# HipGraph/Force2Vec

Hardware: AMD Instinct MI355X
Metric: embedding edges/sec at D=128, option 5 (higher is better)
Workload: dtype f32; 1 GPU; RMAT scale-20 edge-factor 16 (n=1048576, nnz=31404412 directed CSR nonzeros), option 5, D=128, ns=5, lr=0.02, batch=65536; step = 1 epoch; batch=65536, hub_chunk=128, parallelism=1 GPU, recoveries=0, merge_finalize=1

## Files before the change

### force2vec_amd/_lib.py

```python
import ctypes as C
import os

HERE = os.path.dirname(os.path.abspath(__file__))
LIB_PATH = os.path.join(HERE, "libf2v.so")
SELFTEST_LIB_PATH = os.path.join(HERE, "libf2v_selftest.so")

F2V_OK, F2V_EINVAL, F2V_ENODEV, F2V_ENOMEM, F2V_EIO, F2V_ESTATE = 0, -1, -2, -3, -4, -5
INIT_SYMMETRIC, INIT_UNIT = 0, 1
SIM_DOT, SIM_L2, SIM_COSINE = 0, 1, 2
NEAREST_MAX_K = 128
NEAREST_EXCLUDE_SELF, NEAREST_EXCLUDE_NEIGHBOURS = 1, 2
NEAREST_PAD_ID = 0xFFFFFFFF
KMEANS_MAX_K, KMEANS_PIECE = 1024, 64

u32p = C.POINTER(C.c_uint32)
f32p = C.POINTER(C.c_float)


class Stats(C.Structure):
    _fields_ = [("step_launches", C.c_uint64), ("rows", C.c_uint64), ("nnz", C.c_uint64),
                ("algorithmic_bytes", C.c_uint64), ("device_seconds", C.c_double),
                ("hub_rows", C.c_uint64), ("hub_chunks", C.c_uint64), ("compulsory_bytes", C.c_uint64),
                ("snapshot_seconds", C.c_double), ("recoveries", C.c_uint64), ("recovered", C.c_uint32), ("merge_finalize", C.c_uint32)]

# ... 55 lines not shown
    "f2v_push_masks": (C.c_int, [u32p, u32p, C.c_uint32, C.c_uint32, C.c_uint32, u32p, C.c_uint64, u32p]),
    "f2v_push_stats": (C.c_int, [C.c_void_p, C.POINTER(C.c_uint64), C.POINTER(C.c_uint64)]),
    "f2v_read_mtx": (C.c_int, [C.c_char_p, u32p, C.POINTER(C.c_uint64), C.POINTER(u32p), C.POINTER(u32p)]),
    "f2v_free": (None, [C.c_void_p]),
    "f2v_write_embd": (C.c_int, [C.c_char_p, f32p, C.c_uint32, C.c_uint32]),
    "f2v_write_csr_bin": (C.c_int, [C.c_char_p, u32p, u32p, C.c_uint32, C.c_uint64]),
    "f2v_read_csr_bin": (C.c_int, [C.c_char_p, u32p, C.POINTER(C.c_uint64), C.POINTER(u32p), C.POINTER(u32p)]),
    "f2v_write_embd_bin": (C.c_int, [C.c_char_p, f32p, C.c_uint32, C.c_uint32]),
    "f2v_read_embd": (C.c_int, [C.c_char_p, u32p, u32p, C.POINTER(f32p)]),
    "f2v_read_embd_bin": (C.c_int, [C.c_char_p, C.c_uint32, C.c_uint32, f32p]),
    "f2v_output_name": (C.c_int, [C.c_char_p, C.c_char_p, C.c_int, C.c_int, C.c_uint32, C.c_uint32, C.c_uint32, C.c_uint32, C.c_char_p, C.c_size_t]),
    "f2v_rng_create": (C.c_void_p, [C.c_uint32]),
    "f2v_rng_destroy": (None, [C.c_void_p]),
    "f2v_rng_next": (C.c_int, [C.c_void_p]),
    "f2v_rng_jump": (None, [C.c_void_p, C.c_uint64]),
    "f2v_rng_fill": (C.c_int, [C.c_void_p, f32p, C.c_uint64, C.c_int]),
    "f2v_rng_walks": (C.c_int, [C.c_void_p, u32p, u32p, C.c_uint32, C.c_uint64, u32p]),
    "f2v_sm_table": (C.c_int, [f32p]),
    "f2v_diag_ipc_preflight": (C.c_int, [C.c_int, C.c_uint32, C.c_uint32, C.c_char_p, C.c_uint64, C.c_double]),
    "f2v_diag_stream_copy": (C.c_int, [C.c_int, C.c_uint64, C.c_uint32, C.POINTER(C.c_double)]),
    "f2v_diag_gather_rate": (C.c_int, [C.c_int, C.c_uint64, C.c_uint32, C.POINTER(C.c_double)]),
}

TEST_SIGNATURES = {
    "f2v_test_push_attach_local": (C.c_int, [C.c_void_p, C.c_uint32, C.c_uint32, C.POINTER(C.c_void_p)]),
    "f2v_test_gather_calibration": (C.c_int, [C.c_int, C.c_uint32, C.c_uint32]),
    "f2v_test_wave_reduce": (C.c_int, [C.c_int, f32p, C.c_uint32, C.c_uint32, f32p]),
    "f2v_test_withhold_flag": (C.c_int, [C.c_void_p, C.c_uint32]),
    "f2v_test_chain_nowait": (C.c_int, [C.c_void_p, C.c_int]),
    "f2v_test_withhold_row": (C.c_int, [C.c_void_p, C.c_uint32]),
    "f2v_test_stamps": (C.c_int, [C.c_void_p, C.c_int, C.POINTER(C.c_uint64)]),
    "f2v_test_xcd_times": (C.c_int, [C.c_void_p, C.c_int, C.POINTER(C.c_uint64)]),
    "f2v_test_plan_gather": (C.c_int, [C.c_void_p, C.c_uint32, C.c_uint32, C.c_uint32, C.c_uint32, C.POINTER(C.c_double)]),
    "f2v_test_wide_plan_check": (C.c_int, [u32p, u32p, C.c_uint32, C.c_uint64, C.c_uint32, C.c_uint32, C.c_int, C.POINTER(C.c_char_p), C.POINTER(C.c_int64), C.c_uint32, C.POINTER(C.c_uint64)]),
}

PUSH_EXPORT_BYTES = 256
PUSH_MAX_RANKS = 8

_lib = None
_selftest = None


class F2VError(RuntimeError):
    def __init__(self, code, msg):
        super().__init__("libf2v error %d: %s" % (code, msg))
        self.code = code


def lib():
    global _lib
    if _lib is None:
        path = os.environ.get("F2V_LIBRARY", LIB_PATH)
        if not os.path.exists(path):
            raise ImportError("%s is missing: build it with `make` (hipcc --offload-arch=gfx950); "
                              "force2vec_amd has no fallback implementation" % path)
        L = C.CDLL(path)
        for name, (res, args) in SIGNATURES.items():
            if path != LIB_PATH and not hasattr(L, name):
                continue
            fn = getattr(L, name)
            fn.restype = res
            fn.argtypes = args
        _lib = L
    return _lib

# ... 21 lines not shown
```

### force2vec_amd/csrc/f2v_engine.hip

```cpp
#include <hip/hip_runtime.h>

#include <algorithm>
#include <chrono>
#include <cstdio>
#include <cstdlib>
#include <cstring>
#include <functional>
#include <condition_variable>
#include <map>
#include <mutex>
#include <memory>
#include <string>
#include <atomic>
#include <thread>
#include <tuple>
#include <type_traits>
#include <vector>

#include "f2v.h"
#ifdef F2V_TEST_HOOKS
#include "f2v_test.h"
#endif
#include "f2v_internal.h"
#include "f2v_kernels.hip.h"
// ... 107 lines not shown
    std::vector<double> loss_values;
    struct Nearest {
        float *d_Q = nullptr, *d_rq = nullptr, *d_rc = nullptr, *d_scores = nullptr;
        uint32_t *d_qids = nullptr, *d_ids = nullptr;
        unsigned long long *d_ws = nullptr, *d_counts = nullptr;
        size_t q_cap = 0, ws_cap = 0, out_cap = 0;
        hipEvent_t ev[2] = {nullptr, nullptr};
        uint32_t splits = 0, block = 0, chunk = 8192;
        uint32_t lds_allowed = 0;
    } nn;
    int rows_sorted = -1;
    struct Kmeans {
        float *d_C = nullptr, *d_bestC = nullptr, *d_dist = nullptr;
        uint32_t *d_labels = nullptr, *d_bestL = nullptr, *d_order = nullptr, *d_hist = nullptr, *d_counts = nullptr, *d_start = nullptr,
                 *d_pstart = nullptr, *d_changed = nullptr, *d_seed = nullptr, *d_mlabels = nullptr;
        double *d_psum = nullptr, *d_ipart = nullptr, *d_inertia = nullptr;
        unsigned long long *d_tallies = nullptr;
        uint32_t cap_k = 0, cap_nc = 0;
        hipEvent_t ev[2] = {nullptr, nullptr};
        uint32_t block = 0;
        uint32_t lds_allowed = 0;
    } km;
    uint32_t last_wide_width = 0;
    bool last_wide_early = false;
    int last_train_form = 0;
    bool plan_overflow = false;
    uint32_t *h_kerr = nullptr;
#ifdef F2V_TEST_HOOKS
    uint32_t test_withhold_slot = kNoSlot, test_withhold_row = kNoSlot;
    uint32_t test_chain_mode = 0;
    bool test_chain_nowait = false;
    unsigned long long *d_xcd = nullptr;
    unsigned long long *d_stamps = nullptr;
#endif
    bool merge_fin = true, capturing = false;
    int cur = 0;
    bool have_x = false, have_walks = false;
    bool x_invalid = false;
    Rand rng;
    uint32_t chunk = 64, fanin = 32;
    bool chunk_auto = true;
    bool use_quarter = true;
    std::map<std::tuple<uint32_t, uint32_t, int>, Plan> plans;
    std::map<std::tuple<uint32_t, uint32_t, uint32_t, int>, ChainPlan> chains;
    std::vector<WgDesc> h_wg;
    WgDesc *d_wg = nullptr;
    size_t d_wg_cap = 0, d_wg_valid = 0;
    std::map<std::tuple<uint32_t, uint32_t, uint32_t, int>, WidePlan> wides;
    PlanVec<WideDesc> h_wide;
    PlanVec<WJob> h_jobs;
    WideDesc *d_wide = nullptr;
    WJob *d_jobs = nullptr;
    size_t d_wide_cap = 0, d_wide_valid = 0, d_jobs_cap = 0, d_jobs_valid = 0;
    bool wide = true;
    uint32_t wide_max_batch = 2048;
    uint32_t wide_rows = 262144;
    uint32_t wide_order = 0;
    uint32_t wide_phases = 1;
    uint32_t wide_min_width = 0;
    uint32_t wide_epochs = 0, last_wide_epochs = 1;
    float *d_ring = nullptr, *d_ring_partials = nullptr;
    uint32_t *d_ring_flags = nullptr, *d_ring_ready = nullptr;
    uint32_t ring_epochs = 0;
    bool ring_refused = false;
    size_t ring_slots = 0;
    bool wide_single = false;
// ... 1172 lines not shown
    c->stats.compulsory_bytes += plan.compulsory * epochs;
}

void scale_stats(f2v_stats &s, uint64_t epochs, uint64_t per) {
    for (uint64_t *v : {&s.step_launches, &s.rows, &s.nnz, &s.algorithmic_bytes, &s.hub_rows, &s.hub_chunks, &s.compulsory_bytes}) *v = *v / per * epochs;
}

FinalizeArgs finalize_args(const f2v_ctx *c, const StepArgs &a, const FinItem *items, uint32_t n) {
    FinalizeArgs f{};
    f.X = a.X;
    f.partials = c->d_partials;
    f.Xn = a.Xn;
    f.items = items;
    f.n_items = n;
    f.D = c->D;
    f.push = a.push;
    return f;
}

int launch_step(f2v_ctx *c, int math, uint32_t batch_lo, uint32_t batch_hi, uint32_t row_lo, uint32_t row_hi,
                const uint32_t *d_ids, uint32_t ns, float lr, int bs_mode, bool push = false, const uint32_t *push_masks = nullptr) {
    int rc;
    if ((rc = flush_unless_continued(c, batch_lo)) != F2V_OK) return rc;
    const Plan plan = plan_for(c, row_lo, row_hi, math == 7);
    if ((rc = upload_plans(c)) != F2V_OK) return rc;
    StepArgs a{};
    fill_step_args(c, a, math, plan.item_off, c->upd_lo, ns, lr, bs_mode);
    a.sample_ids = d_ids;
    a.batch_lo = batch_lo;
    a.n_items = plan.n_items;
    a.upd_rows = c->upd_hi - c->upd_lo;
#ifdef F2V_TEST_HOOKS
    a.xcd_times = c->d_xcd;
#endif
    push = push && c->push.attached && c->push.world > 1;
    if (push) fill_targets(c, a.push, c->cur ^ 1, batch_lo, push_masks);

    const uint32_t wpb = (uint32_t)c->waves_per_block;
    const uint32_t width = subwave_width(c);
    const bool quarter = width != 0;
    const uint32_t per_wave = items_per_wave(width);
    const uint32_t waves = (plan.n_items + per_wave - 1) / per_wave;
    uint32_t blocks = (waves + wpb - 1) / wpb;
    a.step_blocks = blocks;
    uint32_t tree_nodes = 0;
    for (int lev = 0; lev < plan.n_levels; lev++) tree_nodes += plan.fin_cnt[lev];
    const bool fused_tree = quarter && c->merge_fin && !c->capturing && plan.n_levels >= 1 && blocks > 0;
    if (fused_tree) {
        a.fin_items = c->d_hubs + plan.fin_off[0];
        a.fin_n = tree_nodes;
        arm_waits(c, a, false);
        blocks += (a.fin_n + wpb - 1) / wpb;
    }
    if (blocks == 0) {
    } else if (quarter) {
        rc = dispatch_subwave<16, true>(c, math, width, [&](auto O, auto L, auto N, auto U, auto FL) {
            constexpr int OPT = decltype(O)::value, LPI = decltype(L)::value, NB = decltype(N)::value, UR = decltype(U)::value;
            constexpr bool FULL = decltype(FL)::value;
            if (push) hipLaunchKernelGGL((qstep_kernel<OPT, LPI, NB, UR, true, FULL>), dim3(blocks), dim3(64 * wpb), 0, c->stream, a);
            else hipLaunchKernelGGL((qstep_kernel<OPT, LPI, NB, UR, false, FULL>), dim3(blocks), dim3(64 * wpb), 0, c->stream, a);
        });
        if (rc != F2V_OK) return rc;
    } else {
        rc = dispatch_math_layout(c, math, [&](auto O, auto V, auto E) {
            hipLaunchKernelGGL((step_kernel<decltype(O)::value, decltype(V)::value, decltype(E)::value>), dim3(blocks), dim3(64 * wpb), 0, c->stream, a);
        });
// ... 1969 lines not shown
        }
        hipError_t he = hipIpcOpenMemHandle((void **)&c->push.peer_flags[r], e.flags, hipIpcMemLazyEnablePeerAccess);
        if (he != hipSuccess) {
            c->push.peer_flags[r] = nullptr;
            (void)push_detach(c);
            return fail(F2V_ENODEV, "f2v_push_attach: cannot map the flags of rank %u: %s", r, hipGetErrorString(he));
        }
    }
    c->push.mask_batch = 0;
    c->push.exported = false;
    return F2V_OK;
}

#ifdef F2V_TEST_HOOKS
int f2v_test_withhold_flag(f2v_handle c, uint32_t slot) {
    if (!c) return fail(F2V_EINVAL, "null handle");
    c->test_withhold_slot = slot;
    return F2V_OK;
}

int f2v_test_withhold_row(f2v_handle c, uint32_t row) {
    if (!c) return fail(F2V_EINVAL, "null handle");
    c->test_withhold_row = row;
    return F2V_OK;
}

int f2v_test_chain_nowait(f2v_handle c, int on) {
    if (!c) return fail(F2V_EINVAL, "null handle");
    c->test_chain_nowait = (on & 1) != 0;
    c->test_chain_mode = (uint32_t)on;
    return F2V_OK;
}

int f2v_test_wide_plan_check(const uint32_t *rowptr, const uint32_t *colids, uint32_t n, uint64_t nnz, uint32_t dim, uint32_t batch, int walk,
                             const char *const *names, const int64_t *values, uint32_t n_params, uint64_t *stats_out) {
    if (!rowptr || (!colids && nnz) || n < 2 || dim == 0 || batch == 0) return fail(F2V_EINVAL, "f2v_test_wide_plan_check: bad argument");
    f2v_ctx ctx;
    f2v_ctx *c = &ctx;
    unsigned plan_threads = 0;
    c->n = n; c->nnz = nnz; c->D = dim;
    c->rowptr.assign(rowptr, rowptr + n + 1);
    c->colids.assign(colids, colids + nnz);
    c->chunk = auto_chunk(c, batch);
    static const char *const planner_reads[] = {"hub_chunk", "hub_fanin", "class_cut", "wide_phases", "wide_rounds", "wide_span", "wide_finish", "wide_order", "wide_rows", "wide_min_width"};
    for (uint32_t k = 0; k < n_params; k++) {
        const char *nm = names[k];
        if (!strcmp(nm, "plan_threads")) plan_threads = (unsigned)values[k];
        else if (std::any_of(std::begin(planner_reads), std::end(planner_reads), [&](const char *r) { return !strcmp(r, nm); })) find_param(nm)->put(c, values[k]);
        else return fail(F2V_EINVAL, "f2v_test_wide_plan_check: unknown parameter '%s'", nm);
    }
    if (!wide_usable(c) || subwave_width(c) == 0) return fail(F2V_EINVAL, "f2v_test_wide_plan_check: the wide form does not run this shape");
    const uint32_t nb = (uint32_t)(((uint64_t)n + batch - 1) / batch), K = chain_len(c, batch, true);
    const uint32_t width = wide_width(c, batch), ipb = wide_items_per_block(width), pslots = std::max<uint32_t>(ipb, 32u), F = c->fanin;
    std::vector<uint32_t> finished(n, 0), covered(nnz, 0);
    uint64_t st[7] = {};
    if (plan_threads) wide_plans_for_epoch(c, nb, K, batch, walk != 0, plan_threads);
#define F2V_PLAN_FAIL(...) return fail(F2V_ESTATE, "f2v_test_wide_plan_check: " __VA_ARGS__)
    for (uint32_t b0 = 0; b0 < nb; b0 += K) {
        const WidePlan p = wide_plan_for(c, b0, std::min(K, nb - b0), batch, walk != 0);
        if (c->plan_overflow) F2V_PLAN_FAIL("slot overflow");
        st[0] += p.n_wgs; st[1] += p.n_helpers; st[2] += p.n_finishers; st[3] += p.n_packed; st[4] += p.n_node_wgs; st[5] = std::max<uint64_t>(st[5], p.n_slots);
        std::vector<int64_t> producer(p.n_slots + 1, -1);
        uint32_t last_lo = 0;
        for (uint32_t wgi = 0; wgi < p.n_wgs; wgi++) {
            const WideDesc &d = c->h_wide[p.wg_off + wgi];
            if (d.kind == 0) {
// ... 469 lines not shown
```

### force2vec_amd/csrc/f2v_kernels.hip.h

```cpp
#ifndef F2V_KERNELS_HIP_H_
#define F2V_KERNELS_HIP_H_

#include <hip/hip_runtime.h>
#include <stdint.h>

namespace f2v {
#ifdef F2V_TEST_HOOKS
inline namespace selftest {
#endif

struct Item {
    uint32_t row;
    uint32_t nb;
    uint32_t cnt;
    uint32_t flags;
};
constexpr uint32_t kItemPartial = 1u << 31;
constexpr uint32_t kItemFirst = 1u << 30;
constexpr uint32_t kItemLast = 1u << 29;
constexpr uint32_t kItemSlotMask = (1u << 28) - 1;

struct FinItem {
    uint32_t in_slot, n;
    uint32_t out;
// ... 13 lines not shown
struct StepArgs {
    const float *X;
    float *Xn;
    const uint32_t *rowptr;
    const uint32_t *nbr_ids;
    float *partials;
    const uint32_t *sample_ids;
    const Item *items;
    const float *sm_table;
    uint32_t D;
    uint32_t batch_lo;
    uint32_t n_items;
    uint32_t upd_lo, upd_rows;
    uint32_t ns;
    uint32_t bs_mode;
    uint32_t unit_degi;
    float lr;
    PushTargets push;
    const FinItem *fin_items;
    uint32_t fin_n;
    uint32_t step_blocks;
    uint32_t seq;
    uint32_t *ready;
    uint32_t *err;
    unsigned long long timeout_ticks;
    uint32_t *rowflag;
    uint32_t chain_lo, chain_rows;
#ifdef F2V_TEST_HOOKS
    uint32_t test_withhold_slot;
    unsigned long long *stamps;
    uint32_t test_withhold_row;
    uint32_t test_nowait;
    unsigned long long *xcd_times;
#endif
};
constexpr uint32_t kNoSlot = 0xFFFFFFFFu;

struct FinalizeArgs {
    const float *X;
    float *partials;
    float *Xn;
    const FinItem *items;
    uint32_t n_items;
    uint32_t D;
    PushTargets push;
};

template <int CTRL>
__device__ __forceinline__ float dpp_mov(float v) {
    return __builtin_bit_cast(float, __builtin_amdgcn_update_dpp(0, __builtin_bit_cast(int, v), CTRL, 0xF, 0xF, true));
}

__device__ __forceinline__ float wave_allreduce_tree(float v) {
    v = v + dpp_mov<0xB1>(v);
    v = v + dpp_mov<0x4E>(v);
    v = v + dpp_mov<0x141>(v);
    v = v + dpp_mov<0x140>(v);
    v = v + __builtin_bit_cast(float, __builtin_amdgcn_ds_swizzle(__builtin_bit_cast(int, v), 0x401F));
    const float lo = __builtin_bit_cast(float, __builtin_amdgcn_readlane(__builtin_bit_cast(int, v), 0));
    const float hi = __builtin_bit_cast(float, __builtin_amdgcn_readlane(__builtin_bit_cast(int, v), 32));
    return lo + hi;
}

template <int VEC>
__device__ __forceinline__ float inlane_tree(float (&t)[VEC]) {
#pragma unroll
// ... 489 lines not shown

template <int OPT, int LPI, int NB, bool NEG>
__device__ __forceinline__ void pair_apply_q(const float (&xi)[NB][4], const float4 (&xj4)[NB], float (&Y)[NB][4], float lr,
                                             typename PairCoef<OPT, NEG>::type coef) {
    float xj[NB][4];
#pragma unroll
    for (int b = 0; b < NB; ++b) {
        xj[b][0] = xj4[b].x; xj[b][1] = xj4[b].y; xj[b][2] = xj4[b].z; xj[b][3] = xj4[b].w;
    }
#pragma unroll
    for (int b = 0; b < NB; ++b) {
#pragma unroll
        for (int v = 0; v < 4; ++v) {
            if constexpr (OPT == 5) {
                const float f = clamp_ref((xi[b][v] - xj[b][v]) * coef);
                const float s = lr * f;
                Y[b][v] = Y[b][v] + s;
            } else if constexpr (!NEG) {
                Y[b][v] = (float)((double)xj[b][v] * coef + (double)Y[b][v]);
            } else {
                const float p = coef * xj[b][v];
                Y[b][v] = Y[b][v] - p;
            }
        }
    }
}

template <int OPT, int LPI, int NB, bool NEG>
__device__ __forceinline__ void pair_update_q(const float (&xi)[NB][4], const float4 (&xj4)[NB], float (&Y)[NB][4],
                                              float lr, double c0, const float *table) {
    pair_apply_q<OPT, LPI, NB, NEG>(xi, xj4, Y, lr, pair_coef_q<OPT, LPI, NB, NEG>(xi, xj4, lr, c0, table));
}

__device__ __forceinline__ bool wait_row_slow(const StepArgs &a, const uint32_t *flags, uint32_t j) {
    const uint32_t *f = flags + j;
    const unsigned long long t0 = wall_clock64();
    for (uint32_t spins = 1;; ++spins) {
        __builtin_amdgcn_s_sleep(1);
        if (__hip_atomic_load(f, __ATOMIC_RELAXED, __HIP_MEMORY_SCOPE_AGENT) == a.seq) {
#ifdef F2V_TEST_HOOKS
            if (a.stamps) atomicMax(a.stamps + 4 * (size_t)j + 3, ~wall_clock64());
#endif
            return false;
        }
        if ((spins & 15u) != 0u) continue;
        if (__hip_atomic_load(a.err, __ATOMIC_RELAXED, __HIP_MEMORY_SCOPE_AGENT) != 0u) return true;
        if (wall_clock64() - t0 > a.timeout_ticks) {
            if (__hip_atomic_fetch_add(a.err + 1, 1u, __ATOMIC_RELAXED, __HIP_MEMORY_SCOPE_AGENT) == 0u) {
                a.err[2] = blockIdx.x; a.err[3] = j; a.err[4] = *f; a.err[5] = a.seq; a.err[6] = gridDim.x; a.err[7] = a.batch_lo;
            }
            __hip_atomic_store(a.err, 3u, __ATOMIC_RELAXED, __HIP_MEMORY_SCOPE_AGENT);
            return true;
        }
    }
}

__device__ __forceinline__ bool wait_row_at(const StepArgs &a, const uint32_t *flags, uint32_t j) {
    bool bad = false;
    if (__hip_atomic_load(flags + j, __ATOMIC_RELAXED, __HIP_MEMORY_SCOPE_AGENT) != a.seq) bad = wait_row_slow(a, flags, j);
    asm volatile("" ::: "memory");
    return bad;
}
__device__ __forceinline__ bool wait_row(const StepArgs &a, uint32_t j) { return wait_row_at(a, a.rowflag, j); }

__device__ __forceinline__ const float *row_src(const StepArgs &a, uint32_t j, uint32_t D) {
    return ((j - a.upd_lo) < a.upd_rows ? a.Xn : a.X) + (size_t)j * D;
}

typedef __amdgpu_buffer_rsrc_t rsrc_t;
__device__ __forceinline__ rsrc_t hand_rsrc(const float *base) {
    return __builtin_amdgcn_make_buffer_rsrc(const_cast<float *>(base), 0, -1, 0x00020000);
}
__device__ __forceinline__ float4 load16_agent(rsrc_t r, uint32_t byte_off) {
    const f32x4_t v = __builtin_bit_cast(f32x4_t, __builtin_amdgcn_raw_buffer_load_b128(r, (int)byte_off, 0,  16));
    return make_float4(v.x, v.y, v.z, v.w);
}
struct HandSrc {
    rsrc_t r;
    uint32_t xn_off, x_off, row_bytes;
    __device__ __forceinline__ uint32_t at(uint32_t j, bool second) const { return j * row_bytes + (second ? xn_off : x_off); }
};
__device__ __forceinline__ HandSrc hand_src_window(const StepArgs &a, uint32_t D) {
    HandSrc h;
    h.r = hand_rsrc(a.Xn + (size_t)a.chain_lo * D);
    h.row_bytes = D * 4u;
    h.xn_off = 0u - a.chain_lo * h.row_bytes;
    h.x_off = 0u;
    return h;
}

template <int OPT, int LPI, int NB, bool NEG, int U, bool FULL, bool CHAIN>
__device__ __forceinline__ void qprocess(const StepArgs &a, const HandSrc &hs, const uint32_t *ids, const uint32_t *idle, uint32_t cnt, uint32_t maxcnt,
                                         uint32_t t, uint32_t D, const float (&xi)[NB][4], float (&Y)[NB][4], double c0, const float *table, bool &bad) {
    constexpr bool kAllInFlight = !CHAIN && !(OPT != 5 && !FULL && U == 4);
    if constexpr (kAllInFlight) {
        const uint32_t last = cnt != 0u ? cnt - 1u : 0u;
        const uint32_t *list = cnt != 0u ? ids : idle;
        uint32_t j[U];
#pragma unroll
        for (int u = 0; u < U; ++u) j[u] = list[(uint32_t)u < last ? (uint32_t)u : last];
        for (uint32_t g = 0; g < maxcnt; g += U) {
            float4 xj[U][NB];
#pragma unroll
            for (int u = 0; u < U; ++u) {
                const float *src = row_src(a, j[u], D);
#pragma unroll
                for (int b = 0; b < NB; ++b) {
                    if constexpr (FULL) {
                        xj[u][b] = *reinterpret_cast<const float4 *>(src + t * 4 + 4 * LPI * b);
                    } else {
                        const bool live = 4u * LPI * b + 4u * t < D;
                        const float4 v = *reinterpret_cast<const float4 *>(src + (live ? t * 4 + 4 * LPI * b : 0u));
                        xj[u][b] = live ? v : make_float4(0.f, 0.f, 0.f, 0.f);
                    }
                }
            }
#pragma unroll
            for (int u = 0; u < U; ++u) {
                const uint32_t k = g + U + u;
                j[u] = list[k < last ? k : last];
            }
            asm volatile("" ::: "memory");
#pragma unroll
            for (int u = 0; u < U; ++u) {
                if (g + u < cnt) pair_update_q<OPT, LPI, NB, NEG>(xi, xj[u], Y, a.lr, c0, table);
            }
        }
        return;
    }
    uint32_t j[U];
#pragma unroll
    for (int u = 0; u < U; ++u) j[u] = ((uint32_t)u < cnt) ? ids[u] : 0u;
    for (uint32_t g = 0; g < maxcnt; g += U) {
        float4 xj[U][NB];
#pragma unroll
        for (int u = 0; u < U; ++u) {
            if (g + u < cnt) {
                bool handed = false;
                if constexpr (CHAIN) {
                    handed = (j[u] - a.chain_lo) < a.chain_rows;
                    if (handed) bad = wait_row(a, j[u]) || bad;
                }
                const float *src = row_src(a, j[u], D) + t * 4;
#pragma unroll
                for (int b = 0; b < NB; ++b) {
                    if (!(FULL || 4u * LPI * b + 4u * t < D)) xj[u][b] = make_float4(0.f, 0.f, 0.f, 0.f);
                    else if (CHAIN && handed) xj[u][b] = load16_agent(hs.r, hs.at(j[u], true) + 16u * t + 16u * LPI * b);
                    else xj[u][b] = *reinterpret_cast<const float4 *>(src + 4 * LPI * b);
                }
            }
        }
#pragma unroll
        for (int u = 0; u < U; ++u) j[u] = (g + U + u < cnt) ? ids[g + U + u] : 0u;
#pragma unroll
        for (int u = 0; u < U; ++u) {
            if (g + u < cnt) pair_update_q<OPT, LPI, NB, NEG>(xi, xj[u], Y, a.lr, c0, table);
        }
    }
// ... 185 lines not shown
    if (active) it = a.items[idx];
    else { it.row = 0; it.nb = 0; it.cnt = 0; it.flags = 0; }
    const uint32_t row = it.row;
    const bool partial = (it.flags & kItemPartial) != 0;
    const bool first_chunk = (it.flags & kItemFirst) != 0;
    const bool last_chunk = (it.flags & kItemLast) != 0;

    float xi[NB][4], Y[NB][4];
    {
        const float *src = a.X + (size_t)row * D + t * 4;
#pragma unroll
        for (int b = 0; b < NB; ++b) {
            const float4 v = (FULL || 4u * LPI * b + 4u * t < D) ? *reinterpret_cast<const float4 *>(src + 4 * LPI * b) : make_float4(0.f, 0.f, 0.f, 0.f);
            xi[b][0] = v.x; xi[b][1] = v.y; xi[b][2] = v.z; xi[b][3] = v.w;
        }
    }
    double c0 = 0.0;
    if constexpr (OPT == 5) {
#pragma unroll
        for (int b = 0; b < NB; ++b)
#pragma unroll
            for (int v = 0; v < 4; ++v) Y[b][v] = 0.0f;
    } else {
#pragma unroll
        for (int b = 0; b < NB; ++b)
#pragma unroll
            for (int v = 0; v < 4; ++v) Y[b][v] = first_chunk ? xi[b][v] : 0.0f;
        const uint32_t gdeg = a.rowptr[row + 1] - a.rowptr[row];
        const float degi = a.unit_degi ? 1.0f : (float)(1.0 / (double)(gdeg + 1u));
        c0 = (double)(a.lr * degi);
    }

    bool bad = false;
    const uint32_t *idle = &a.items[active ? idx : IPW * w].row;
    qprocess<OPT, LPI, NB, false, U, FULL, CHAIN>(a, hs, a.nbr_ids + it.nb, idle, it.cnt, wave_max_of_items<LPI>(it.cnt), t, D, xi, Y, c0, table, bad);
    if (lds_samples) {
        if (active && last_chunk) {
            for (uint32_t sidx = 0; sidx < a.ns; ++sidx) {
                float4 xs[NB];
#pragma unroll
                for (int b = 0; b < NB; ++b) xs[b] = smp[sidx][LPI * b + t];
                pair_update_q<OPT, LPI, NB, true>(xi, xs, Y, a.lr, c0, table);
            }
        }
    } else {
        const uint32_t scnt = (active && last_chunk) ? a.ns : 0u;
        const uint32_t sbase = a.bs_mode ? (row - a.batch_lo) : 0u;
        qprocess<OPT, LPI, NB, true, U, FULL, CHAIN>(a, hs, a.sample_ids + sbase, idle, scnt, wave_max_of_items<LPI>(scnt), t, D, xi, Y, c0, table, bad);
    }

    if (CHAIN && __builtin_amdgcn_ballot_w64(bad) != 0ull) {
        return;
    }
    if (active) {
        float *out = (partial ? a.partials + (size_t)(it.flags & kItemSlotMask) * D : a.Xn + (size_t)row * D) + t * 4;
        float4 v[NB];
#pragma unroll
        for (int b = 0; b < NB; ++b) {
            if (OPT == 5 && !partial)
                v[b] = make_float4(xi[b][0] + Y[b][0], xi[b][1] + Y[b][1], xi[b][2] + Y[b][2], xi[b][3] + Y[b][3]);
            else
                v[b] = make_float4(Y[b][0], Y[b][1], Y[b][2], Y[b][3]);
            if (!FULL && !(4u * LPI * b + 4u * t < D)) continue;
            if ((partial && a.fin_items) || CHAIN) store16_agent(out + 4 * LPI * b, v[b]);
            else *reinterpret_cast<float4 *>(out + 4 * LPI * b) = v[b];
        }
        if constexpr (PUSH) {
            if (!partial) {
                const uint32_t others = ((1u << a.push.world) - 1u) & ~(1u << a.push.self);
                const uint32_t m = (a.push.masks ? a.push.masks[row] : others) & others;
#pragma unroll
                for (int q = 0; q < kMaxRanks; ++q) {
                    if (m & (1u << q)) {
                        float *dst = a.push.peer[q] + (size_t)(row - a.push.row_base) * D + t * 4;
#pragma unroll
                        for (int b = 0; b < NB; ++b)
                            if (FULL || 4u * LPI * b + 4u * t < D) store16_system(dst + 4 * LPI * b, v[b]);
                    }
                }
            }
        }
    }
    if constexpr (PUSH) __builtin_amdgcn_s_waitcnt(0);
    if constexpr (CHAIN) {
        __builtin_amdgcn_s_waitcnt(0);
#ifdef F2V_TEST_HOOKS
        if (active && !partial && t == 0u && row != a.test_withhold_row)
#else
        if (active && !partial && t == 0u)
#endif
            __hip_atomic_store(a.rowflag + row, a.seq, __ATOMIC_RELAXED, __HIP_MEMORY_SCOPE_AGENT);
#ifdef F2V_TEST_HOOKS
        if (a.stamps && active && !partial && t == 0u) a.stamps[4 * (size_t)row + 2] = wall_clock64();
#endif
    }
    if (a.fin_items) {
        __builtin_amdgcn_s_waitcnt(0);
#ifdef F2V_TEST_HOOKS
        if ((it.flags & kItemSlotMask) == a.test_withhold_slot) return;
#endif
        if (active && partial && t == 0u) __hip_atomic_store(a.ready + (it.flags & kItemSlotMask), a.seq, __ATOMIC_RELAXED, __HIP_MEMORY_SCOPE_AGENT);
#ifdef F2V_TEST_HOOKS
        if (a.stamps && active && partial && it.cnt != 0u && t == 0u) atomicMax(a.stamps + 4 * (size_t)row, wall_clock64());
#endif
    }
}

template <int OPT, int LPI, int NB, int U, bool PUSH = false, bool FULL = true>
__global__ __launch_bounds__(256) void qstep_kernel(const StepArgs a) {
#ifdef F2V_TEST_HOOKS
    const unsigned long long t0 = a.xcd_times ? wall_clock64() : 0ull;
#endif
    qstep_body<OPT, LPI, NB, U, PUSH, FULL, false>(a, blockIdx.x);
#ifdef F2V_TEST_HOOKS
    if (a.xcd_times && threadIdx.x == 0u) {
        uint32_t id;
        asm volatile("s_getreg_b32 %0, hwreg(HW_REG_XCC_ID, 0, 4)" : "=s"(id));
        const unsigned long long t1 = wall_clock64();
        atomicMax(a.xcd_times + (id & 7u), t1);
        atomicMin(a.xcd_times + 8u + (id & 7u), t0);
        atomicAdd(a.xcd_times + 16u + (id & 7u), t1 - t0);
        atomicAdd(a.xcd_times + 24u + (id & 7u), 1ull);
    }
#endif
}

struct WgDesc {
    uint32_t lo;
    uint32_t item_off;
    uint32_t n_items;
    uint32_t step_blocks;
    uint32_t fin_off, fin_n;
    uint32_t index;
    uint32_t blk;
};
struct ChainArgs {
    StepArgs base;
    const WgDesc *wg;
    const uint32_t *ids;
    uint32_t ids_stride;
};

// ... 424 lines not shown
                    }
                }
            }
            return false;
        };
        qprocess_pre<OPT, LPI, NB, U, FULL, MODE == 0>(a, hs, a.nbr_ids + it.nb, cnt, wave_max_of_items<LPI>(cnt), t, D, xi, Y, c0, table, bad, jpre,
                                            a.nbr_ids + itn.nb, (itn.flags & kItemIdle) ? 0u : itn.cnt, between, prev_flags);
        if constexpr (!EARLY) (void)stage_late();
        if (quit) return;
        if (lds_samples) {
            if (!idle && last_chunk) {
                if constexpr (EARLY) {
#pragma unroll
                    for (int sidx = 0; sidx < (int)kLdsSamples; ++sidx) {
                        if ((uint32_t)sidx < a.ns) {
                            float4 xs[NB];
#pragma unroll
                            for (int b = 0; b < NB; ++b) xs[b] = smp[sidx][LPI * b + t];
                            pair_apply_q<OPT, LPI, NB, true>(xi, xs, Y, a.lr, cs[sidx]);
                        }
                    }
                } else {
                    for (uint32_t sidx = 0; sidx < a.ns; ++sidx) {
                        float4 xs[NB];
#pragma unroll
                        for (int b = 0; b < NB; ++b) xs[b] = smp[sidx][LPI * b + t];
                        pair_update_q<OPT, LPI, NB, true>(xi, xs, Y, a.lr, c0, table);
                    }
                }
            }
        } else {
            const uint32_t scnt = (!idle && last_chunk) ? a.ns : 0u;
            const uint32_t sbase = a.bs_mode ? (row - a.batch_lo) : 0u;
            qprocess<OPT, LPI, NB, true, U, FULL, true>(a, hs, a.sample_ids + sbase, nullptr, scnt, wave_max_of_items<LPI>(scnt), t, D, xi, Y, c0, table, bad);
        }
        const bool wave_bad = __builtin_amdgcn_ballot_w64(bad) != 0ull;
        if (wave_bad) wg_bad = 1u;
        if (!idle && !wave_bad) {
            if (direct) {
                float *out = a.Xn + (size_t)row * D + t * 4;
#pragma unroll
                for (int b = 0; b < NB; ++b) {
                    if (!FULL && !(4u * LPI * b + 4u * t < D)) continue;
                    const float4 v = OPT == 5 ? make_float4(xi[b][0] + Y[b][0], xi[b][1] + Y[b][1], xi[b][2] + Y[b][2], xi[b][3] + Y[b][3])
                                              : make_float4(Y[b][0], Y[b][1], Y[b][2], Y[b][3]);
                    store16_agent(out + 4 * LPI * b, v);
                }
            } else {
#pragma unroll
                for (int b = 0; b < NB; ++b) slots[it.flags & kItemPieceSlot][LPI * b + t] = make_float4(Y[b][0], Y[b][1], Y[b][2], Y[b][3]);
#ifdef F2V_TEST_HOOKS
                if (a.stamps && t == 0u) atomicMax(a.stamps + 4 * (size_t)row, wall_clock64());
#endif
            }
        }
        if (__builtin_amdgcn_ballot_w64(!idle && direct) != 0ull) {
            __builtin_amdgcn_s_waitcnt(0);
            if (!idle && direct && !wave_bad && t == 0u) {
#ifdef F2V_TEST_HOOKS
                if (row != a.test_withhold_row)
#endif
                __hip_atomic_store(a.rowflag + row, a.seq, __ATOMIC_RELAXED, __HIP_MEMORY_SCOPE_AGENT);
#ifdef F2V_TEST_HOOKS
                if (a.stamps) a.stamps[4 * (size_t)row + 2] = wall_clock64();
#endif
            }
        }
// ... 497 lines not shown
```

Baseline: 18.09 billion edges/s.

## Batch option-5 coefficient division across quad lanes and raise step kernel occupancy

For option 5, the per-pair distance reductions for four neighbours (or eight negative samples) are computed first. Lanes then select one sum each via bitmasks so the double-precision divide for the coefficient runs once per lane instead of once per pair, and the results are broadcast back with DPP. Negative samples read from LDS get the same two-pass treatment. It also adds a min-waves launch bound for option-5 step kernels, adds asm register barriers to steer codegen, and adds a test-only stub mode that skips the interaction math. The risks are extra register pressure from holding distances across the batch and possible spills under the tighter launch bound.

```diff
diff --git a/force2vec_amd/_lib.py b/force2vec_amd/_lib.py
--- a/force2vec_amd/_lib.py
+++ b/force2vec_amd/_lib.py
@@ -111,6 +111,7 @@
     "f2v_test_stamps": (C.c_int, [C.c_void_p, C.c_int, C.POINTER(C.c_uint64)]),
     "f2v_test_xcd_times": (C.c_int, [C.c_void_p, C.c_int, C.POINTER(C.c_uint64)]),
     "f2v_test_plan_gather": (C.c_int, [C.c_void_p, C.c_uint32, C.c_uint32, C.c_uint32, C.c_uint32, C.POINTER(C.c_double)]),
+    "f2v_test_interaction_stub": (C.c_int, [C.c_void_p, C.c_uint32]),
     "f2v_test_wide_plan_check": (C.c_int, [u32p, u32p, C.c_uint32, C.c_uint64, C.c_uint32, C.c_uint32, C.c_int, C.POINTER(C.c_char_p), C.POINTER(C.c_int64), C.c_uint32, C.POINTER(C.c_uint64)]),
 }
 
diff --git a/force2vec_amd/csrc/f2v_engine.hip b/force2vec_amd/csrc/f2v_engine.hip
--- a/force2vec_amd/csrc/f2v_engine.hip
+++ b/force2vec_amd/csrc/f2v_engine.hip
@@ -163,6 +163,7 @@
     bool test_chain_nowait = false;
     unsigned long long *d_xcd = nullptr;
     unsigned long long *d_stamps = nullptr;
+    uint32_t test_stub = 0;
 #endif
     bool merge_fin = true, capturing = false;
     int cur = 0;
@@ -1401,6 +1402,7 @@
     a.upd_rows = c->upd_hi - c->upd_lo;
 #ifdef F2V_TEST_HOOKS
     a.xcd_times = c->d_xcd;
+    a.test_stub = c->test_stub;
 #endif
     push = push && c->push.attached && c->push.world > 1;
     if (push) fill_targets(c, a.push, c->cur ^ 1, batch_lo, push_masks);
@@ -3436,6 +3438,12 @@
     return F2V_OK;
 }
 
+int f2v_test_interaction_stub(f2v_handle c, uint32_t mode) {
+    if (!c) return fail(F2V_EINVAL, "null handle");
+    c->test_stub = mode & 3u;
+    return F2V_OK;
+}
+
 int f2v_test_wide_plan_check(const uint32_t *rowptr, const uint32_t *colids, uint32_t n, uint64_t nnz, uint32_t dim, uint32_t batch, int walk,
                              const char *const *names, const int64_t *values, uint32_t n_params, uint64_t *stats_out) {
     if (!rowptr || (!colids && nnz) || n < 2 || dim == 0 || batch == 0) return fail(F2V_EINVAL, "f2v_test_wide_plan_check: bad argument");
diff --git a/force2vec_amd/csrc/f2v_kernels.hip.h b/force2vec_amd/csrc/f2v_kernels.hip.h
--- a/force2vec_amd/csrc/f2v_kernels.hip.h
+++ b/force2vec_amd/csrc/f2v_kernels.hip.h
@@ -69,6 +69,7 @@
     uint32_t test_withhold_row;
     uint32_t test_nowait;
     unsigned long long *xcd_times;
+    uint32_t test_stub;
 #endif
 };
 constexpr uint32_t kNoSlot = 0xFFFFFFFFu;
@@ -624,6 +625,126 @@
     pair_apply_q<OPT, LPI, NB, NEG>(xi, xj4, Y, lr, pair_coef_q<OPT, LPI, NB, NEG>(xi, xj4, lr, c0, table));
 }
 
+typedef float f32x2_t __attribute__((ext_vector_type(2)));
+
+template <bool NEG>
+__device__ __forceinline__ float coef5(float a) {
+    if constexpr (NEG) return (float)(2.0 / ((double)a * (1.0 + (double)a)));
+    else return (float)(-2.0 / (1.0 + (double)a));
+}
+
+template <int LPI, int NB>
+__device__ __forceinline__ float pair_dist_q(const float (&xi)[NB][4], const float4 (&xj4)[NB], f32x2_t (&d)[NB][2]) {
+    float bs[NB];
+#pragma unroll
+    for (int b = 0; b < NB; ++b) {
+        d[b][0] = f32x2_t{xi[b][0], xi[b][1]} - f32x2_t{xj4[b].x, xj4[b].y};
+        d[b][1] = f32x2_t{xi[b][2], xi[b][3]} - f32x2_t{xj4[b].z, xj4[b].w};
+        const f32x2_t s0 = d[b][0] * d[b][0], s1 = d[b][1] * d[b][1];
+        float t01 = s0.x + s0.y;
+        asm("" : "+v"(t01));
+        bs[b] = item_allreduce_tree<LPI>(t01 + (s1.x + s1.y));
+        asm("" : "+v"(bs[b]));
+    }
+    if constexpr (NB == 1) return bs[0];
+    else if constexpr (NB == 2) return bs[0] + bs[1];
+    else return (bs[0] + bs[1]) + (bs[2] + bs[3]);
+}
+
+template <int N>
+struct LaneSel { uint32_t m[N == 4 ? 2 : 3]; };
+template <int N>
+__device__ __forceinline__ LaneSel<N> lane_sel(uint32_t t) {
+    LaneSel<N> s;
+#pragma unroll
+    for (int k = 0; k < (N == 4 ? 2 : 3); ++k) {
+        s.m[k] = 0u - ((t >> k) & 1u);
+        asm volatile("" : "+v"(s.m[k]));
+    }
+    return s;
+}
+
+template <int N, bool NEG>
+__device__ __forceinline__ void shared_coef5(const float (&a)[N], const LaneSel<N> &sel, float (&cf)[N]) {
+    static_assert(N == 4 || N == 8, "a quad, or the two quads of a half row");
+    uint32_t m[N];
+#pragma unroll
+    for (int k = 0; k < N; ++k) m[k] = __builtin_bit_cast(uint32_t, a[k]);
+#pragma unroll
+    for (int s = 1, l = 0; s < N; s <<= 1, ++l) {
+#pragma unroll
+        for (int k = 0; k + s < N; k += 2 * s) m[k] = (m[k + s] & sel.m[l]) | (m[k] & ~sel.m[l]);
+    }
+    const int c = __builtin_bit_cast(int, coef5<NEG>(__builtin_bit_cast(float, m[0])));
+    int q[4];
+    q[0] = __builtin_amdgcn_update_dpp(0, c, 0x00, 0xF, 0xF, true);
+    q[1] = __builtin_amdgcn_update_dpp(0, c, 0x55, 0xF, 0xF, true);
+    q[2] = __builtin_amdgcn_update_dpp(0, c, 0xAA, 0xF, 0xF, true);
+    q[3] = __builtin_amdgcn_update_dpp(0, c, 0xFF, 0xF, 0xF, true);
+#pragma unroll
+    for (int u = 0; u < N; ++u) {
+        if constexpr (N == 4) cf[u] = __builtin_bit_cast(float, q[u]);
+        else cf[u] = __builtin_bit_cast(float, u < 4 ? __builtin_amdgcn_update_dpp(q[u & 3], q[u & 3], 0x141, 0xF, 0xA, false)
+                                                     : __builtin_amdgcn_update_dpp(q[u & 3], q[u & 3], 0x141, 0xF, 0x5, false));
+    }
+}
+
+template <int NB>
+__device__ __forceinline__ void pair_apply5_q(const f32x2_t (&d)[NB][2], float (&Y)[NB][4], float lr, float coef) {
+#pragma unroll
+    for (int b = 0; b < NB; ++b) {
+#pragma unroll
+        for (int h = 0; h < 2; ++h) {
+            f32x2_t f = d[b][h] * coef;
+            f.x = clamp_ref(f.x);
+            f.y = clamp_ref(f.y);
+            const f32x2_t s = lr * f;
+            Y[b][2 * h] = Y[b][2 * h] + s.x;
+            Y[b][2 * h + 1] = Y[b][2 * h + 1] + s.y;
+        }
+    }
+}
+
+template <int LPI, int NB>
+__device__ __forceinline__ void lds_samples5_q(const float4 (*smp)[LPI * NB], uint32_t ns, uint32_t t, const float (&xi)[NB][4], float (&Y)[NB][4], float lr) {
+    float sum[8], cf[8];
+#pragma unroll
+    for (uint32_t sidx = 0; sidx < 8u; ++sidx) {
+        sum[sidx] = 1.0f;
+        if (sidx < ns) {
+            float4 xs[NB];
+            f32x2_t d[NB][2];
+#pragma unroll
+            for (int b = 0; b < NB; ++b) xs[b] = smp[sidx][LPI * b + t];
+            sum[sidx] = pair_dist_q<LPI, NB>(xi, xs, d);
+        }
+    }
+    shared_coef5<8, true>(sum, lane_sel<8>(t), cf);
+#pragma unroll
+    for (uint32_t sidx = 0; sidx < 8u; ++sidx) {
+        if (sidx < ns) {
+            f32x2_t d[NB][2];
+#pragma unroll
+            for (int b = 0; b < NB; ++b) {
+                const float4 xs = smp[sidx][LPI * b + t];
+                d[b][0] = f32x2_t{xi[b][0], xi[b][1]} - f32x2_t{xs.x, xs.y};
+                d[b][1] = f32x2_t{xi[b][2], xi[b][3]} - f32x2_t{xs.z, xs.w};
+            }
+            pair_apply5_q<NB>(d, Y, lr, cf[sidx]);
+        }
+    }
+}
+
+#ifdef F2V_TEST_HOOKS
+template <int NB>
+__device__ __forceinline__ void stub_update_q(const float4 (&xj4)[NB], float (&Y)[NB][4]) {
+#pragma unroll
+    for (int b = 0; b < NB; ++b) {
+        Y[b][0] = Y[b][0] + xj4[b].x; Y[b][1] = Y[b][1] + xj4[b].y; Y[b][2] = Y[b][2] + xj4[b].z; Y[b][3] = Y[b][3] + xj4[b].w;
+    }
+}
+#endif
+
 __device__ __forceinline__ bool wait_row_slow(const StepArgs &a, const uint32_t *flags, uint32_t j) {
     const uint32_t *f = flags + j;
     const unsigned long long t0 = wall_clock64();
@@ -682,12 +803,13 @@
 }
 
 template <int OPT, int LPI, int NB, bool NEG, int U, bool FULL, bool CHAIN>
-__device__ __forceinline__ void qprocess(const StepArgs &a, const HandSrc &hs, const uint32_t *ids, const uint32_t *idle, uint32_t cnt, uint32_t maxcnt,
+__device__ __forceinline__ void qprocess(const StepArgs &a, const HandSrc &hs, const uint32_t *ids, uint32_t idle, uint32_t cnt, uint32_t maxcnt,
                                          uint32_t t, uint32_t D, const float (&xi)[NB][4], float (&Y)[NB][4], double c0, const float *table, bool &bad) {
     constexpr bool kAllInFlight = !CHAIN && !(OPT != 5 && !FULL && U == 4);
     if constexpr (kAllInFlight) {
         const uint32_t last = cnt != 0u ? cnt - 1u : 0u;
-        const uint32_t *list = cnt != 0u ? ids : idle;
+        asm volatile("" : "+v"(idle));
+        const uint32_t *list = cnt != 0u ? ids : &a.items[idle].row;
         uint32_t j[U];
 #pragma unroll
         for (int u = 0; u < U; ++u) j[u] = list[(uint32_t)u < last ? (uint32_t)u : last];
@@ -713,9 +835,41 @@
                 j[u] = list[k < last ? k : last];
             }
             asm volatile("" ::: "memory");
-#pragma unroll
-            for (int u = 0; u < U; ++u) {
-                if (g + u < cnt) pair_update_q<OPT, LPI, NB, NEG>(xi, xj[u], Y, a.lr, c0, table);
+#ifdef F2V_TEST_HOOKS
+            if (a.test_stub & 1u) {
+#pragma unroll
+                for (int u = 0; u < U; ++u)
+                    if (g + u < cnt) stub_update_q<NB>(xj[u], Y);
+                continue;
+            }
+#endif
+            if constexpr (OPT == 5 && !NEG && NB * U <= 8) {
+                const LaneSel<4> sel = lane_sel<4>(t);
+#pragma unroll
+                for (int h = 0; h < U; h += 4) {
+                    f32x2_t d[4][NB][2];
+                    float sum[4], cf[4];
+#pragma unroll
+                    for (int u = 0; u < 4; ++u) {
+#pragma unroll
+                        for (int b = 0; b < NB; ++b) {
+                            f32x4_t v = {xj[h + u][b].x, xj[h + u][b].y, xj[h + u][b].z, xj[h + u][b].w};
+                            asm volatile("" : "+v"(v));
+                            xj[h + u][b] = make_float4(v.x, v.y, v.z, v.w);
+                        }
+                        sum[u] = pair_dist_q<LPI, NB>(xi, xj[h + u], d[u]);
+                    }
+                    shared_coef5<4, NEG>(sum, sel, cf);
+#pragma unroll
+                    for (int u = 0; u < 4; ++u) {
+                        if (g + h + u < cnt) pair_apply5_q<NB>(d[u], Y, a.lr, cf[u]);
+                    }
+                }
+            } else {
+#pragma unroll
+                for (int u = 0; u < U; ++u) {
+                    if (g + u < cnt) pair_update_q<OPT, LPI, NB, NEG>(xi, xj[u], Y, a.lr, c0, table);
+                }
             }
         }
         return;
@@ -967,14 +1121,27 @@
     }
 
     bool bad = false;
-    const uint32_t *idle = &a.items[active ? idx : IPW * w].row;
+    const uint32_t idle = active ? idx : IPW * w;
     qprocess<OPT, LPI, NB, false, U, FULL, CHAIN>(a, hs, a.nbr_ids + it.nb, idle, it.cnt, wave_max_of_items<LPI>(it.cnt), t, D, xi, Y, c0, table, bad);
     if (lds_samples) {
         if (active && last_chunk) {
-            for (uint32_t sidx = 0; sidx < a.ns; ++sidx) {
+            bool together = OPT == 5 && !CHAIN && LPI >= kLdsSamples;
+#ifdef F2V_TEST_HOOKS
+            together = together && (a.test_stub & 2u) == 0u;
+#endif
+            if constexpr (OPT == 5 && !CHAIN && LPI >= kLdsSamples) {
+                if (together) lds_samples5_q<LPI, NB>(smp, a.ns, t, xi, Y, a.lr);
+            }
+            for (uint32_t sidx = 0; !together && sidx < a.ns; ++sidx) {
                 float4 xs[NB];
 #pragma unroll
                 for (int b = 0; b < NB; ++b) xs[b] = smp[sidx][LPI * b + t];
+#ifdef F2V_TEST_HOOKS
+                if (a.test_stub & 2u) {
+                    stub_update_q<NB>(xs, Y);
+                    continue;
+                }
+#endif
                 pair_update_q<OPT, LPI, NB, true>(xi, xs, Y, a.lr, c0, table);
             }
         }
@@ -987,8 +1154,15 @@
     if (CHAIN && __builtin_amdgcn_ballot_w64(bad) != 0ull) {
         return;
     }
+    uint32_t ts = t, row_out = row;
+    if constexpr (OPT == 5) {
+        uint32_t tid = threadIdx.x;
+        asm volatile("" : "+v"(tid));
+        ts = tid & (LPI - 1u);
+        asm("" : "+v"(row_out));
+    }
     if (active) {
-        float *out = (partial ? a.partials + (size_t)(it.flags & kItemSlotMask) * D : a.Xn + (size_t)row * D) + t * 4;
+        float *out = (partial ? a.partials + (size_t)(it.flags & kItemSlotMask) * D : a.Xn + (size_t)row_out * D) + ts * 4;
         float4 v[NB];
 #pragma unroll
         for (int b = 0; b < NB; ++b) {
@@ -996,7 +1170,7 @@
                 v[b] = make_float4(xi[b][0] + Y[b][0], xi[b][1] + Y[b][1], xi[b][2] + Y[b][2], xi[b][3] + Y[b][3]);
             else
                 v[b] = make_float4(Y[b][0], Y[b][1], Y[b][2], Y[b][3]);
-            if (!FULL && !(4u * LPI * b + 4u * t < D)) continue;
+            if (!FULL && !(4u * LPI * b + 4u * ts < D)) continue;
             if ((partial && a.fin_items) || CHAIN) store16_agent(out + 4 * LPI * b, v[b]);
             else *reinterpret_cast<float4 *>(out + 4 * LPI * b) = v[b];
         }
@@ -1007,10 +1181,10 @@
 #pragma unroll
                 for (int q = 0; q < kMaxRanks; ++q) {
                     if (m & (1u << q)) {
-                        float *dst = a.push.peer[q] + (size_t)(row - a.push.row_base) * D + t * 4;
+                        float *dst = a.push.peer[q] + (size_t)(row - a.push.row_base) * D + ts * 4;
 #pragma unroll
                         for (int b = 0; b < NB; ++b)
-                            if (FULL || 4u * LPI * b + 4u * t < D) store16_system(dst + 4 * LPI * b, v[b]);
+                            if (FULL || 4u * LPI * b + 4u * ts < D) store16_system(dst + 4 * LPI * b, v[b]);
                     }
                 }
             }
@@ -1020,13 +1194,13 @@
     if constexpr (CHAIN) {
         __builtin_amdgcn_s_waitcnt(0);
 #ifdef F2V_TEST_HOOKS
-        if (active && !partial && t == 0u && row != a.test_withhold_row)
+        if (active && !partial && ts == 0u && row != a.test_withhold_row)
 #else
-        if (active && !partial && t == 0u)
+        if (active && !partial && ts == 0u)
 #endif
             __hip_atomic_store(a.rowflag + row, a.seq, __ATOMIC_RELAXED, __HIP_MEMORY_SCOPE_AGENT);
 #ifdef F2V_TEST_HOOKS
-        if (a.stamps && active && !partial && t == 0u) a.stamps[4 * (size_t)row + 2] = wall_clock64();
+        if (a.stamps && active && !partial && ts == 0u) a.stamps[4 * (size_t)row + 2] = wall_clock64();
 #endif
     }
     if (a.fin_items) {
@@ -1034,15 +1208,22 @@
 #ifdef F2V_TEST_HOOKS
         if ((it.flags & kItemSlotMask) == a.test_withhold_slot) return;
 #endif
-        if (active && partial && t == 0u) __hip_atomic_store(a.ready + (it.flags & kItemSlotMask), a.seq, __ATOMIC_RELAXED, __HIP_MEMORY_SCOPE_AGENT);
-#ifdef F2V_TEST_HOOKS
-        if (a.stamps && active && partial && it.cnt != 0u && t == 0u) atomicMax(a.stamps + 4 * (size_t)row, wall_clock64());
-#endif
-    }
-}
-
+        if (active && partial && ts == 0u) __hip_atomic_store(a.ready + (it.flags & kItemSlotMask), a.seq, __ATOMIC_RELAXED, __HIP_MEMORY_SCOPE_AGENT);
+#ifdef F2V_TEST_HOOKS
+        if (a.stamps && active && partial && it.cnt != 0u && ts == 0u) atomicMax(a.stamps + 4 * (size_t)row, wall_clock64());
+#endif
+    }
+}
+
+#ifdef F2V_TEST_HOOKS
+template <int OPT, int NB, int U>
+constexpr int kStepWaves = 1;
+#else
+template <int OPT, int NB, int U>
+constexpr int kStepWaves = (OPT == 5 && NB * U <= 8) ? 5 : 1;
+#endif
 template <int OPT, int LPI, int NB, int U, bool PUSH = false, bool FULL = true>
-__global__ __launch_bounds__(256) void qstep_kernel(const StepArgs a) {
+__global__ __launch_bounds__(256, (kStepWaves<OPT, NB, U>)) void qstep_kernel(const StepArgs a) {
 #ifdef F2V_TEST_HOOKS
     const unsigned long long t0 = a.xcd_times ? wall_clock64() : 0ull;
 #endif
@@ -1533,7 +1714,7 @@
         } else {
             const uint32_t scnt = (!idle && last_chunk) ? a.ns : 0u;
             const uint32_t sbase = a.bs_mode ? (row - a.batch_lo) : 0u;
-            qprocess<OPT, LPI, NB, true, U, FULL, true>(a, hs, a.sample_ids + sbase, nullptr, scnt, wave_max_of_items<LPI>(scnt), t, D, xi, Y, c0, table, bad);
+            qprocess<OPT, LPI, NB, true, U, FULL, true>(a, hs, a.sample_ids + sbase, 0u, scnt, wave_max_of_items<LPI>(scnt), t, D, xi, Y, c0, table, bad);
         }
         const bool wave_bad = __builtin_amdgcn_ballot_w64(bad) != 0ull;
         if (wave_bad) wg_bad = 1u;
```

After: 20.82 billion edges/s, median of 6. 1.15x the previous value.
